# leggedrobotics/wild_visual_navigation

Measured on AMD Instinct MI355X. Metric: frames/sec (448x448 DINO-ViT-S/8 + seg + MLP train-step), higher is better.
Workload: dtype fp16 + e5m2-MX-correction linears (a w = a_h w_h + 2^-12 (a_h8 w_l8 + a_l8 w_h8); ~16 significand bits per product) + f16 attention products (two-plane q in the first six blocks), fp32 accumulate / residual (<= 1e-3 parity mode)

## Files before the change

include/wvn_hip.h:

```cpp
#ifndef WVN_HIP_H
#define WVN_HIP_H
#include <stddef.h>
#ifdef __cplusplus
extern "C" {
#endif

#define WVN_MAX_DEPTH 32
#define WVN_PREC_F32 0
#define WVN_PREC_BF16 1
#define WVN_PREC_X3 2
#define WVN_PREC_FP8 3
#define WVN_PREC_F16 4

#define WVN_PREC_MIX 5

int wvn_version(void);

#define WVN_VIT_MLP_FUSED 1
#define WVN_VIT_QKV_FUSED 2
#define WVN_VIT_FUSE_ANY_SIZE 4
#define WVN_VIT_NO_PROJ_IN_MLP 8
#define WVN_VIT_NO_LN_HANDOVER 16
#define WVN_VIT_NO_A384_X3 32
#define WVN_VIT_X3_NO_A384 64
// ... 302 lines not shown

size_t wvn_rnvp_train_param_count(const wvn_rnvp_desc* d);
size_t wvn_rnvp_train_workspace_bytes(const wvn_rnvp_desc* d, long long R);
size_t wvn_rnvp_train_pack_bytes(const wvn_rnvp_desc* d);
int wvn_rnvp_train_pack(const wvn_rnvp_desc* d, const float* params, const void* packed, void* train_packed, void* stream);
int wvn_rnvp_train_phase_a(const wvn_rnvp_desc* d, const void* packed, const float* x, int ldx, long long R, float* score,
                           double* stats, void* workspace, size_t workspace_bytes, void* stream);
int wvn_rnvp_train_phase_b(const wvn_rnvp_desc* d, const void* packed, const void* train_packed, long long R, const double* stats,
                           float* grads, void* workspace, size_t workspace_bytes, void* stream);
int wvn_rnvp_train_phase_c(const wvn_rnvp_desc* d, float* params, const float* grads, float* adam_m, float* adam_v, int step, float lr,
                           const double* stats, int method, double* conf_state, float* losses, const float* mask,
                           const long long* perm, void* packed, void* train_packed, void* stream);

size_t wvn_segment_predict_workspace_bytes(const wvn_mlp_desc* d, int B, int S);
int wvn_segment_predict(const wvn_mlp_desc* d, const float* params, const float* feat, int ld_row, long long ld_frame,
                        int B, int S, const void* seg, int seg_bytes, int H, int W, float mean, float std, float std_factor,
                        const float* conf_state, float* trav, float* conf, float* loss_reco, void* workspace,
                        size_t workspace_bytes, void* stream);

size_t wvn_wire_bytes(int H, int W, int S, int D);
int wvn_wire_pack(const void* seg, int seg_is_i64, const float* feat, int ldf, void* out, int H, int W, int S, int D, void* stream);
int wvn_wire_unpack(const void* in, long long* seg_i64, int* seg_i32, float* feat, int H, int W, int S, int D, void* stream);

int wvn_debug_gemm_bf16_timed(const void* A, int lda, const void* W, int ldw, const float* bias, void* C, int ldc, int M,
                              int N, int K, int epi, long long* dbg, void* stream);
int wvn_debug_gemm_a384_x3(const void* A, const void* A_lo, int lda, const void* W, const void* W_lo, const float* bias, void* C,
                           void* C_lo, int ldc, int M, int N, int epi, long long* dbg, void* stream);
int wvn_debug_gemm_n384_x3(const void* A, const void* A_lo, int lda, const void* W, const void* W_lo, const float* bias, const float* ls,
                           float* C, int ldc, int M, int K, long long* dbg, void* stream);
int wvn_debug_mlp_x3_frag(const void* xn, const void* xn_lo, const void* W1, const void* W1_lo, const float* b1, void* hid, void* hid_lo,
                          const void* W2p, const float* b2, float* x, int M, int F, long long* dbg1, long long* dbg2, void* stream);
int wvn_debug_gemm_n384_mx(const void* A_h, const void* A_l8, const void* A_h8, const void* Wp, const float* bias, const float* ls, float* C,
                           int ldc, int M, int K, long long* dbg, void* stream);
int wvn_debug_mlp_mx(const float* x, int ldx, const float* ln_stats, const float* ln_g, const float* ln_b, const void* W1p, const float* b1,
                     void* hid_h, void* hid_l8, void* hid_h8, const void* W2p, const float* b2, float* xout, int M, int F, long long* dbg1,
                     long long* dbg2, void* stream);
int wvn_debug_qkv_mx(const float* x, int ldx, const float* ln_stats, const float* ln_g, const float* ln_b, const void* Wp, const float* bias, void* q,
                     void* q_lo, void* k, void* vt, int heads, int npad, int ntok_s, float q_scale, int M, long long* dbg, void* stream);
int wvn_debug_stego_head_fused(const float* x, int ldx, const float* stats, const float* ln_g, const float* ln_b, const void* w_cat, const float* b_cat,
                               void* hid, void* hid_lo, float* code, int ld_code, int frames, int npatch, int ntok_s, void* stream);
int wvn_debug_f16_saturate(const float* in, void* out_f16, int n, void* stream);
int wvn_debug_attention_timing(long long* dbg);
int wvn_debug_attention_variant(int variant);
int wvn_debug_attention_planes(const void* q, const void* q_lo, const void* k, const void* vt, void* out, void* out_lo, int B, int heads,
                               int ntok, int ntok_s, int npad, int out_frag, int qsplit_form, void* stream);
int wvn_debug_n384_pair(int on);
int wvn_debug_kmeans_assign_form(int form);
int wvn_debug_kmeans_linear_rows(int rows);

int wvn_debug_kmeans_screen_stats(unsigned long long* out, int reset);
int wvn_debug_qkv_fused_timing(long long* dbg);
int wvn_debug_mlp_fused_timing(long long* dbg);
int wvn_debug_gemm_n384(const void* A, int lda, const void* W, int ldw, const float* bias, float* C, int ldc, int M, int K,
                        void* stream);


size_t wvn_dense_crf_workspace_bytes(int B, int H, int W, int K);
int wvn_dense_crf(const float* logits1, int K1, long long s1b, long long s1c, long long s1p, const float* logits2, int K2, long long s2b,
                  long long s2c, long long s2p, const unsigned char* image, int B, int H, int W, int iterations, float pos_w, float pos_xy_std,
                  float bi_w, float bi_xy_std, float bi_rgb_std, int* labels, int* nseg_last, float* probs, float* debug, void* workspace,
                  size_t workspace_bytes, void* stream);
int wvn_crf_image(const void* frame, int frame_u8, int B, int src_h, int src_w, const int* rows, const int* cols, int out_h, int out_w,
                  unsigned char* out, void* stream);

size_t wvn_dense_crf_permutohedral_workspace_bytes(int B, int H, int W, int K);
int wvn_dense_crf_permutohedral(const float* logits1, int K1, long long s1b, long long s1c, long long s1p, const float* logits2, int K2,
// ... 14 lines not shown
```

wild_visual_navigation_amd/_lib.py:

```python
import ctypes as C
import os
import threading

import torch

_HERE = os.path.dirname(os.path.abspath(__file__))
LIB_PATH = os.environ.get("WVN_LIB_PATH") or os.path.join(_HERE, "lib", "libwvn_hip.so")
if os.environ.get("WVN_LIB_PATH"):
    import sys as _sys

    print(f"[wild_visual_navigation_amd] WVN_LIB_PATH is set: loading {LIB_PATH} instead of the in-tree build", file=_sys.stderr)

WVN_MAX_DEPTH = 32
PREC_F32, PREC_BF16, PREC_X3, PREC_FP8, PREC_F16, PREC_MIX = 0, 1, 2, 3, 4, 5
VIT_MLP_FUSED = 1
VIT_QKV_FUSED = 2
VIT_FUSE_ANY_SIZE = 4
VIT_NO_PROJ_IN_MLP = 8
VIT_NO_LN_HANDOVER = 16
VIT_NO_A384_X3 = 32
VIT_NO_MX = 1024


def vit_qsplit_blocks(n: int) -> int:
# ... 50 lines not shown


class RnvpDesc(C.Structure):
    _fields_ = [("D", C.c_int), ("h", C.c_int), ("flows", C.c_int)]


MLP_KIND_DOUBLE = 1


_lib = None
_lock = threading.Lock()

_i, _f, _p, _ll, _sz = C.c_int, C.c_float, C.c_void_p, C.c_longlong, C.c_size_t
_SIGNATURES = {
    "wvn_version": ([], _i),
    "wvn_vit_workspace_bytes": ([_p, _i], _sz),
    "wvn_vit_forward": ([_p, _p, _i, _p, _p, _i, _p, _sz, _p], _i),
    "wvn_vit_forward_u8": ([_p, _p, _i, _p, _p, _i, _p, _sz, _p], _i),
    "wvn_vit_forward_frames": ([_p, _p, _i, _i, _i, _p, _p, _i, _p, _p, _i, _p, _sz, _p], _i),
    "wvn_vit_forward_frames_pair": ([_p, _p, _i, _i, _i, _p, _p, _p, _i, _p, _p, _i, _p, _sz, _p], _i),
    "wvn_vit_forward_frames_head": ([_p, _p, _i, _i, _i, _p, _p, _p, _i, _p, _p, _sz, _p], _i),
    "wvn_debug_stego_head_fused": ([_p, _i, _p, _p, _p, _p, _p, _p, _p, _p, _i, _i, _i, _i, _p], _i),
    "wvn_resize_nearest_crop": ([_p, _p, _ll, _i, _i, _p, _p, _i, _i, _i, _p], _i),
    "wvn_prof_enable": ([_i], _i),
    "wvn_prof_collect": ([_p, _p], _i),
    "wvn_gemm_bf16": ([_p, _i, _p, _i, _p, _p, _i, _i, _i, _i, _i, _p], _i),
    "wvn_debug_attention_variant": ([_i], _i),
    "wvn_debug_attention_planes": ([_p, _p, _p, _p, _p, _p, _i, _i, _i, _i, _i, _i, _i, _p], _i),
    "wvn_debug_kmeans_assign_form": ([_i], _i),
    "wvn_debug_kmeans_screen_stats": ([_p, _i], _i),
    "wvn_debug_mlp_x3_frag": ([_p, _p, _p, _p, _p, _p, _p, _p, _p, _p, _i, _i, _p, _p, _p], _i),
    "wvn_debug_gemm_n384_x3": ([_p, _p, _i, _p, _p, _p, _p, _p, _i, _i, _i, _p, _p], _i),
    "wvn_debug_gemm_n384_mx": ([_p, _p, _p, _p, _p, _p, _p, _i, _i, _i, _p, _p], _i),
    "wvn_debug_mlp_mx": ([_p, _i, _p, _p, _p, _p, _p, _p, _p, _p, _p, _p, _p, _i, _i, _p, _p, _p], _i),
    "wvn_debug_qkv_mx": ([_p, _i, _p, _p, _p, _p, _p, _p, _p, _p, _p, _i, _i, _i, _f, _i, _p, _p], _i),
    "wvn_debug_gemm_a384_x3": ([_p, _p, _i, _p, _p, _p, _p, _p, _i, _i, _i, _i, _p, _p], _i),
    "wvn_stream_create_cu_mask": ([_p, _p, _i], _i),
    "wvn_stream_destroy": ([_p], _i),
    "wvn_debug_qkv_fused_timing": ([_p], _i),
    "wvn_debug_mlp_fused_timing": ([_p], _i),
    "wvn_qkv_fused": ([_p, _i, _p, _p, _f, _p, _p, _p, _p, _p, _i, _i, _i, _f, _i, _p], _i),
    "wvn_proj_mlp_fused": ([_p, _i, _p, _p, _p, _p, _p, _f, _p, _p, _p, _p, _p, _p, _i, _i, _i, _p], _i),
    "wvn_mlp_fused": ([_p, _i, _p, _p, _f, _p, _p, _p, _p, _p, _p, _i, _i, _i, _p], _i),
    "wvn_gemm_f16": ([_p, _i, _p, _i, _p, _p, _i, _i, _i, _i, _i, _p], _i),
    "wvn_qkv_fused_f16": ([_p, _i, _p, _p, _f, _p, _p, _p, _p, _p, _i, _i, _i, _f, _i, _p], _i),
    "wvn_proj_mlp_resident": ([_p, _i, _p, _p, _p, _p, _f, _p, _p, _p, _p, _p, _i, _i, _i, _p, _p, _f, _p, _p], _i),
    "wvn_proj_mlp_resident_f16": ([_p, _i, _p, _p, _p, _p, _f, _p, _p, _p, _p, _p, _i, _i, _i, _p, _p, _f, _p, _p], _i),
    "wvn_qkv_prenorm": ([_p, _p, _p, _p, _p, _p, _i, _i, _i, _f, _i, _p], _i),
    "wvn_qkv_prenorm_f16": ([_p, _p, _p, _p, _p, _p, _i, _i, _i, _f, _i, _p], _i),
    "wvn_proj_mlp_fused_f16": ([_p, _i, _p, _p, _p, _p, _p, _f, _p, _p, _p, _p, _p, _p, _i, _i, _i, _p], _i),
    "wvn_mlp_fused_f16": ([_p, _i, _p, _p, _f, _p, _p, _p, _p, _p, _p, _i, _i, _i, _p], _i),
    "wvn_attention_f16": ([_p, _p, _p, _p, _i, _i, _i, _i, _f, _p], _i),
    "wvn_gemm_x3": ([_p, _p, _i, _p, _p, _i, _p, _p, _p, _i, _i, _i, _i, _i, _p], _i),
    "wvn_quantize_rows_fp8": ([_p, _i, _i, _p, _i, _p, _i, _i, _p], _i),
    "wvn_layernorm_fp8": ([_p, _p, _p, _p, _i, _p, _i, _i, _f, _p], _i),
    "wvn_gemm_fp8": ([_p, _i, _p, _i, _p, _p, _p, _p, _i, _i, _i, _i, _i, _p], _i),
    "wvn_gemm_a768_fp8": ([_p, _i, _p, _p, _p, _p, _p, _p, _i, _i, _i, _i, _p, _p, _p, _i, _i, _i, _f, _p], _i),
    "wvn_gemm_fp8_mx": ([_p, _i, _p, _p, _i, _p, _p, _p, _p, _i, _i, _i, _i, _i, _p], _i),
    "wvn_split_planes": ([_p, _i, _p, _p, _i, _i, _i, _p], _i),
    "wvn_attention_x3": ([_p, _p, _p, _p, _p, _p, _p, _p, _i, _i, _i, _i, _f, _p], _i),
    "wvn_gemm_f32": ([_p, _i, _i, _p, _i, _i, _p, _p, _i, _i, _i, _i, _i, _p, _i, _p], _i),
    "wvn_layernorm": ([_p, _p, _p, _p, _i, _i, _i, _f, _p], _i),
    "wvn_attention_bf16": ([_p, _p, _p, _p, _i, _i, _i, _i, _f, _p], _i),
    "wvn_attention_f32": ([_p, _p, _p, _p, _i, _i, _i, _i, _f, _p], _i),
    "wvn_patchify": ([_p, _p, _i, _i, _i, _i, _p], _i),
    "wvn_patchify_u8": ([_p, _p, _i, _i, _i, _p], _i),
# ... 127 lines not shown
```

wild_visual_navigation_amd/csrc/api.hip:

```cpp
#include <math.h>
#include <string.h>

#include "../../include/wvn_hip.h"

#include "common.h"
#include "wvn_internal.h"

#define RET_IF(x)            \
  do {                       \
    int rc__ = (x);          \
    if (rc__ != WVN_OK) return rc__; \
  } while (0)

extern "C" {

int wvn_version(void) { return 101; }

size_t wvn_vit_workspace_bytes(const wvn_vit_model* m, int batch) {
  if (!m || batch <= 0) return 0;
  return wvn_vit_workspace_bytes_impl(m, batch);
}

int wvn_vit_forward(const wvn_vit_model* m, const float* img, int batch, float* tokens_f32, void* tokens_lowp,
                    int ld_lowp, void* workspace, size_t workspace_bytes, void* stream) {
// ... 190 lines not shown
int wvn_debug_qkv_fused_timing(long long* dbg) { g_qkv_fused_dbg = dbg; return WVN_OK; }
int wvn_stream_create_cu_mask(void** stream, const unsigned int* mask, int words) {
  if (!stream || !mask || words <= 0) return WVN_ERR_ARG;
  hipStream_t st = nullptr;
  const hipError_t e = hipExtStreamCreateWithCUMask(&st, (uint32_t)words, mask);
  if (e != hipSuccess) return (int)e;
  *stream = (void*)st;
  return WVN_OK;
}
int wvn_stream_destroy(void* stream) {
  if (!stream) return WVN_ERR_ARG;
  const hipError_t e = hipStreamDestroy((hipStream_t)stream);
  return e == hipSuccess ? WVN_OK : (int)e;
}

int wvn_debug_gemm_a384_x3(const void* A, const void* A_lo, int lda, const void* W, const void* W_lo, const float* bias, void* C,
                           void* C_lo, int ldc, int M, int N, int epi, long long* dbg, void* stream) {
  if (epi != EPI_GELU_BF16 && epi != EPI_RESID_F32) return WVN_ERR_ARG;
  return wvn_gemm_a384_x3_launch(wvn_desc_a384(A, A_lo, lda, W, W_lo, bias, C, C_lo, ldc, M, N, dbg), epi, (hipStream_t)stream);
}
int wvn_debug_gemm_n384_x3(const void* A, const void* A_lo, int lda, const void* W, const void* W_lo, const float* bias, const float* ls,
                           float* C, int ldc, int M, int K, long long* dbg, void* stream) {
  return wvn_gemm_n384_x3_launch(wvn_desc_n384(A, A_lo, lda, W, W_lo, bias, ls, C, ldc, M, K, nullptr, dbg), EPI_RESID_F32, (hipStream_t)stream);
}
int wvn_debug_mlp_x3_frag(const void* xn, const void* xn_lo, const void* W1, const void* W1_lo, const float* b1, void* hid, void* hid_lo,
                          const void* W2p, const float* b2, float* x, int M, int F, long long* dbg1, long long* dbg2, void* stream) {
  RET_IF(wvn_gemm_a384_x3_launch(wvn_desc_a384(xn, xn_lo, 384, W1, W1_lo, b1, hid, hid_lo, F, M, F, dbg1), EPI_GELU_FRAG, (hipStream_t)stream));
  return wvn_gemm_n384_x3_frag_launch(wvn_desc_n384(hid, hid_lo, F, W2p, nullptr, b2, nullptr, x, 384, M, F, nullptr, dbg2), EPI_RESID_F32, (hipStream_t)stream);
}
int wvn_debug_gemm_n384_mx(const void* A_h, const void* A_l8, const void* A_h8, const void* Wp, const float* bias, const float* ls, float* C,
                           int ldc, int M, int K, long long* dbg, void* stream) {
  return wvn_gemm_n384_mx_launch(wvn_desc_n384(A_h, A_l8, K, Wp, nullptr, bias, ls, C, ldc, M, K, nullptr, dbg, A_h8), EPI_RESID_F32, (hipStream_t)stream);
}
int wvn_debug_mlp_mx(const float* x, int ldx, const float* ln_stats, const float* ln_g, const float* ln_b, const void* W1p, const float* b1,
                     void* hid_h, void* hid_l8, void* hid_h8, const void* W2p, const float* b2, float* xout, int M, int F, long long* dbg1,
                     long long* dbg2, void* stream) {
  GemmBf16Params p1 = wvn_desc_a384(nullptr, nullptr, 0, W1p, nullptr, b1, hid_h, hid_l8, F, M, F, dbg1, hid_h8);
  wvn_desc_ln_on_load(p1, x, ldx, ln_stats, ln_g, ln_b);
  RET_IF(wvn_gemm_a384_mx_launch(p1, EPI_GELU_FRAG, (hipStream_t)stream));
  if (!W2p) return WVN_OK;
  return wvn_gemm_n384_mx_launch(wvn_desc_n384(hid_h, hid_l8, F, W2p, nullptr, b2, nullptr, xout, 384, M, F, nullptr, dbg2, hid_h8), EPI_RESID_F32, (hipStream_t)stream);
}
int wvn_debug_qkv_mx(const float* x, int ldx, const float* ln_stats, const float* ln_g, const float* ln_b, const void* Wp, const float* bias, void* q,
                     void* q_lo, void* k, void* vt, int heads, int npad, int ntok_s, float q_scale, int M, long long* dbg, void* stream) {
  GemmBf16Params p = wvn_desc_a384(nullptr, nullptr, 0, Wp, nullptr, bias, nullptr, nullptr, 0, M, 3 * heads * 64, dbg);
  wvn_desc_ln_on_load(p, x, ldx, ln_stats, ln_g, ln_b);
  wvn_desc_qkv_epilogue(p, q, k, vt, heads, npad, 0, ntok_s, q_scale, 1, q_lo);
  return wvn_gemm_a384_mx_launch(p, EPI_QKV, (hipStream_t)stream);
}
int wvn_debug_n384_pair(int on) {
  if (on >= 32) { wvn_gemm_a384_mx_set_form(on - 32); return WVN_OK; }
  wvn_gemm_n384_x3_set_pair(on);
  return WVN_OK;
}
int wvn_debug_kmeans_screen_stats(unsigned long long* out, int reset) { return out ? wvn_kmeans_pixels_screen_stats(out, reset) : WVN_ERR_ARG; }
int wvn_debug_kmeans_assign_form(int form) { wvn_kmeans_pixels_set_assign_form(form); return WVN_OK; }
int wvn_debug_attention_variant(int v) { wvn_attention_bf16_set_variant(v); wvn_attention_bf16_set_variant_f16(v); return WVN_OK; }
int wvn_debug_attention_planes(const void* q, const void* q_lo, const void* k, const void* vt, void* out, void* out_lo, int B, int heads, int ntok,
                               int ntok_s, int npad, int out_frag, int qsplit_form, void* stream) {
  if (!q || !k || !vt || !out || B < 1 || heads < 1 || ntok < 1 || ntok_s < ntok || ntok_s > npad) return WVN_ERR_ARG;
  if (qsplit_form < 0 || qsplit_form > 2 || (qsplit_form == 0) != (q_lo == nullptr)) return WVN_ERR_ARG;
  if (out_frag < 0 || out_frag > 2 || (out_frag != 0 && (!out_lo || heads != 6))) return WVN_ERR_ARG;
  return wvn_attention_bf16_launch_f16((const bf16_t*)q, (const bf16_t*)k, (const bf16_t*)vt, (bf16_t*)out, B, heads, ntok, ntok_s, npad, 0.f,
                                       (hipStream_t)stream, (bf16_t*)out_lo, (const bf16_t*)q_lo, out_frag, qsplit_form);
}

int wvn_debug_gemm_bf16_timed(const void* A, int lda, const void* W, int ldw, const float* bias, void* C, int ldc, int M,
                              int N, int K, int epi, long long* dbg, void* stream) {
  if (epi < 0 || epi > EPI_ACCUM_F32 || !C) return WVN_ERR_ARG;
  GemmBf16Params p{};
  p.A = (const bf16_t*)A; p.lda = lda; p.W = (const bf16_t*)W; p.ldw = ldw; p.bias = bias; p.C = C; p.ldc = ldc;
  p.M = M; p.N = N; p.K = K; p.dbg = dbg;
  return wvn_gemm_bf16_launch(p, epi, (hipStream_t)stream);
}

int wvn_debug_gemm_n384(const void* A, int lda, const void* W, int ldw, const float* bias, float* C, int ldc, int M, int K,
                        void* stream) {
  GemmBf16Params p{};
  p.A = (const bf16_t*)A; p.lda = lda; p.W = (const bf16_t*)W; p.ldw = ldw; p.bias = bias; p.C = C; p.ldc = ldc;
  p.M = M; p.N = 384; p.K = K;
  return wvn_gemm_n384_launch(p, EPI_RESID_F32, (hipStream_t)stream, nullptr, 1);
}

// ... 583 lines not shown
```

wild_visual_navigation_amd/csrc/gemm_n384_x3.hip:

```cpp
#include <type_traits>

#include "common.h"
#include "wvn_internal.h"

namespace {

constexpr int NN = 384;
constexpr int NTILE = NN / 32;
constexpr int BKS = 16;
constexpr int BM = 128;
constexpr int NS = 4;
constexpr int W_PLANE = NN * BKS * 2;
constexpr int A_PLANE = BM * BKS * 2;
constexpr int A_OFF = 2 * W_PLANE;
constexpr int STAGE_BYTES = 2 * W_PLANE + 2 * A_PLANE;
constexpr int RING_BYTES = NS * STAGE_BYTES;
constexpr int STG_PITCH = 132;
constexpr int STG_BYTES = 32 * STG_PITCH * 4;
constexpr int BIAS_OFF = RING_BYTES;
constexpr int LS_OFF = BIAS_OFF + NN * 4;
constexpr int LDS_BYTES = LS_OFF + NN * 4;
constexpr int WP = 6, AP = 2;

struct N384X3Params {
// ... 529 lines not shown
            __builtin_amdgcn_sched_group_barrier(0x008, 1, 0);
            __builtin_amdgcn_sched_group_barrier(0x100, 1, 0);
            __builtin_amdgcn_sched_group_barrier(0x010, 1, 0);
            __builtin_amdgcn_sched_group_barrier(0x002, 2, 0);
          }
          __builtin_amdgcn_sched_barrier(0);
        }
        if (i + PD < nk) load_a(i + PD, jj);
        __builtin_amdgcn_sched_barrier(0);
        if constexpr (TIMING) { t_wait += c1 - c0; t_steps += (long long)__builtin_amdgcn_s_memtime() - c1; }
      }
    }
    long long e0 = 0;
    if constexpr (TIMING) e0 = (long long)__builtin_amdgcn_s_memtime();
    asm volatile("s_waitcnt vmcnt(0)" ::: "memory");
    n384_pair_epilogue(acc, smem, wave, lane, rg, ch, m0w, rs_c, p.ldc, bias_l, ls_l, p.stats, p.eps, p.M);
    if constexpr (TIMING) t_epi += (long long)__builtin_amdgcn_s_memtime() - e0;
  }
  if constexpr (TIMING) {
    if (lane == 0 && p.dbg && ch == 0) {
      long long* d = p.dbg + ((size_t)blockIdx.x * 4 + rg) * 4;
      d[0] = t_wait; d[1] = t_steps; d[2] = t_epi; d[3] = (long long)__builtin_amdgcn_s_memtime() - t_start;
    }
  }
}

typedef __attribute__((ext_vector_type(8))) int i32x8_t;
typedef __attribute__((ext_vector_type(8))) _Float16 f16x8_t;
constexpr int MXD = 2;
constexpr int MX_SC_ONE = 0x7f7f7f7f, MX_SC_RES = 0x73737373;

struct N384MXExtra { unsigned a_l8_off; };

template <bool TIMING, int VAR = 0>
__global__ __launch_bounds__(512, 1) void gemm_n384_mx_pair_kernel(N384X3Params p, N384MXExtra ex) {
  wvn_fp16_saturate();
  extern __shared__ __attribute__((aligned(16))) unsigned char smem[];
  const int tid = threadIdx.x, lane = tid & 63;
  const int wave = __builtin_amdgcn_readfirstlane(tid >> 6);
  const int rg = wave & 3, ch = wave >> 2;
  const int l31 = lane & 31, hi = lane >> 5;
  const int nk = p.K / BKS;
  const int nmac = p.K / 64;
  const float* bias_l = (const float*)(smem + PBIAS_OFF);
  const float* ls_l = (const float*)(smem + PLS_OFF);
  for (int i = tid; i < NN; i += 512) {
    ((float*)(smem + PBIAS_OFF))[i] = p.bias ? p.bias[i] : 0.f;
    ((float*)(smem + PLS_OFF))[i] = p.ls ? p.ls[i] : 1.f;
  }
  const __amdgpu_buffer_rsrc_t rs_w = __builtin_amdgcn_make_buffer_rsrc((void*)p.W, 0, (unsigned)((size_t)4 * NN * p.K), 0x00020000);
  const size_t mpad = (size_t)(p.M + 31) / 32 * 32;
  const __amdgpu_buffer_rsrc_t rs_a = __builtin_amdgcn_make_buffer_rsrc((void*)p.A, 0, (unsigned)(ex.a_l8_off + mpad * p.K), 0x00020000);
  const __amdgpu_buffer_rsrc_t rs_c = __builtin_amdgcn_make_buffer_rsrc((void*)p.C, 0, (unsigned)((size_t)p.M * p.ldc * 4), 0x00020000);
  const unsigned wv0 = (unsigned)(wave * PFW * 1024 + lane * 16);
  const unsigned rdw = l31 * 32 + ((hi ^ ((l31 >> 3) & 1)) << 4) + ch * 6 * 1024;

  long long t_wait = 0, t_steps = 0, t_epi = 0;
  const long long t_start = TIMING ? (long long)__builtin_amdgcn_s_memtime() : 0;
  const int nrb = (p.M + BM - 1) / BM;
  for (int rb = blockIdx.x; rb < nrb; rb += gridDim.x) {
    const int m0w = rb * BM + rg * 32;
    const unsigned a_base = __builtin_amdgcn_readfirstlane((unsigned)((size_t)(m0w >> 5) * p.K * 64));
    const unsigned a8_base = __builtin_amdgcn_readfirstlane((unsigned)((size_t)(m0w >> 5) * p.K * 32));
    auto piece_w = [&](int i, int u) {
      unsigned char* st = smem + (i % PNS) * FSTAGE;
      __builtin_amdgcn_raw_ptr_buffer_load_lds(rs_w, (__attribute__((address_space(3))) void*)(st + (wave * PFW + u) * 1024), 16, wv0 + u * 1024,
                                               __builtin_amdgcn_readfirstlane((unsigned)i * FSTAGE), 0, 0);
    };
    u32x4_t ah[MXD][4], a8[MXD][2][2];
    auto load_ah = [&](int c, int slot) {
#pragma unroll
      for (int s = 0; s < 4; ++s)
        ah[slot][s] = __builtin_amdgcn_raw_buffer_load_b128(rs_a, lane * 16, __builtin_amdgcn_readfirstlane(a_base + (unsigned)(c * 4 + s) * 1024), 0);
    };
    auto load_a8 = [&](int c, int slot) {
#pragma unroll
      for (int x = 0; x < 2; ++x)
        a8[slot][1][x] = __builtin_amdgcn_raw_buffer_load_b128(rs_a, lane * 16, __builtin_amdgcn_readfirstlane(a8_base + ex.a_l8_off + (unsigned)(c * 2 + x) * 1024), 0);
    };
    auto derive_h8 = [&](int slot) {
      typedef __attribute__((ext_vector_type(2))) short s16x2_t;
      typedef __attribute__((ext_vector_type(2))) _Float16 h2_t;
#pragma unroll
      for (int sfr = 0; sfr < 4; ++sfr) {
        uint32_t d[2] = {0, 0};
#pragma unroll
        for (int e = 0; e < 4; ++e) {
          const uint32_t pr = ah[slot][sfr][e];
          const s16x2_t o = __builtin_bit_cast(s16x2_t, d[e >> 1]);
          d[e >> 1] = __builtin_bit_cast(uint32_t, (e & 1) ? __builtin_amdgcn_cvt_scalef32_pk_bf8_f16(o, __builtin_bit_cast(h2_t, pr), 1.0f, true)
                                                           : __builtin_amdgcn_cvt_scalef32_pk_bf8_f16(o, __builtin_bit_cast(h2_t, pr), 1.0f, false));
        }
        a8[slot][0][sfr >> 1][2 * (sfr & 1)] = d[0];
        a8[slot][0][sfr >> 1][2 * (sfr & 1) + 1] = d[1];
      }
    };
    __syncthreads();
#pragma unroll
    for (int c = 0; c < MXD; ++c) {
      load_ah(c, c);
      __builtin_amdgcn_sched_barrier(0);
      load_a8(c, c);
      __builtin_amdgcn_sched_barrier(0);
    }
#pragma unroll
    for (int i0 = 0; i0 < PNS - 1; ++i0)
      if (i0 < nk) {
#pragma unroll
        for (int u = 0; u < PFW; ++u) piece_w(i0, u);
      }

    f32x16_t acc[NTILE / 2];
#pragma unroll
    for (int t = 0; t < NTILE / 2; ++t)
#pragma unroll
      for (int r = 0; r < 16; ++r) acc[t][r] = 0.f;

    u32x4_t wq[2][2][2];
    asm volatile("s_waitcnt vmcnt(%0)" ::"n"((PNS - 2) * PFW) : "memory");
    __builtin_amdgcn_s_barrier();
#pragma unroll
    for (int x = 0; x < 2; ++x)
#pragma unroll
      for (int t = 0; t < 2; ++t) wq[0][x][t] = *(const u32x4_t*)(smem + rdw + x * W_PLANE + t * 1024);
    for (int ib = 0; ib < nk; ib += 4 * MXD) {
#pragma unroll
      for (int jj = 0; jj < 4 * MXD; ++jj) {
        const int i = ib + jj;
        const int kind = jj & 3, slot = jj >> 2;
        long long c0 = 0, c1 = 0;
        if constexpr (TIMING) c0 = (long long)__builtin_amdgcn_s_memtime();
        if constexpr (VAR != 4) {
          constexpr int W3 = (PNS - 3) * PFW;
          if (jj == 0) { if (i == 0) asm volatile("s_waitcnt vmcnt(%0)" ::"n"(W3) : "memory"); else asm volatile("s_waitcnt vmcnt(%0)" ::"n"(W3 + 6) : "memory"); }
          else if (jj == 1) { if (i == 1) asm volatile("s_waitcnt vmcnt(%0)" ::"n"(W3) : "memory"); else asm volatile("s_waitcnt vmcnt(%0)" ::"n"(W3 + 2) : "memory"); }
          else if (jj == 2) { if (i == 2) asm volatile("s_waitcnt vmcnt(%0)" ::"n"(W3 + 4) : "memory"); else asm volatile("s_waitcnt vmcnt(%0)" ::"n"(W3 + 6) : "memory"); }
          else if ((jj & 3) == 0) asm volatile("s_waitcnt vmcnt(%0)" ::"n"(W3 + 6) : "memory");
          else if ((jj & 3) == 1) asm volatile("s_waitcnt vmcnt(%0)" ::"n"(W3 + 2) : "memory");
          else if ((jj & 3) == 2) asm volatile("s_waitcnt vmcnt(%0)" ::"n"(W3 + 6) : "memory");
          else asm volatile("s_waitcnt vmcnt(%0)" ::"n"(W3 + 4) : "memory");
          __builtin_amdgcn_s_barrier();
        }
        if constexpr (TIMING) c1 = (long long)__builtin_amdgcn_s_memtime();
        __builtin_amdgcn_sched_barrier(0);
        const unsigned char* st = smem + (i % PNS) * FSTAGE;
        const unsigned char* st1 = smem + ((i + 1) % PNS) * FSTAGE;
        const int s0 = jj & 1;
#pragma unroll
        for (int pr = 0; pr < NTILE / 4; ++pr) {
          const int cur = (s0 + pr) & 1, nx = cur ^ 1;
          if constexpr (!(VAR & 1) || VAR == 4) piece_w(i + PNS - 1, pr);
          const unsigned char* src = pr + 1 < NTILE / 4 ? st + (2 * pr + 2) * 1024 : st1;
#pragma unroll
          for (int x = 0; x < 2; ++x)
#pragma unroll
            for (int t = 0; t < 2; ++t) wq[nx][x][t] = *(const u32x4_t*)(src + rdw + x * W_PLANE + t * 1024);
          if (kind == 1 && pr == 0) derive_h8(slot);
          if (kind < 2) {
// ... 1 lines not shown
            for (int x = 0; x < 2; ++x)
#pragma unroll
              for (int t = 0; t < 2; ++t)
                acc[2 * pr + t] = __builtin_amdgcn_mfma_f32_32x32x16_f16(__builtin_bit_cast(f16x8_t, wq[cur][x][t]), __builtin_bit_cast(f16x8_t, ah[slot][2 * kind + x]),
                                                                         acc[2 * pr + t], 0, 0, 0);
#pragma unroll
            for (int n = 0; n < 4; ++n) {
              __builtin_amdgcn_sched_group_barrier(0x008, 1, 0);
              __builtin_amdgcn_sched_group_barrier(0x100, 1, 0);
              __builtin_amdgcn_sched_group_barrier(0x010, 1, 0);
              __builtin_amdgcn_sched_group_barrier(0x002, 2, 0);
            }
          } else {
            const u32x4_t a0 = a8[slot][kind - 2][0], a1 = a8[slot][kind - 2][1];
            const i32x8_t av = {(int)a0[0], (int)a0[1], (int)a0[2], (int)a0[3], (int)a1[0], (int)a1[1], (int)a1[2], (int)a1[3]};
#pragma unroll
            for (int t = 0; t < 2; ++t) {
              const u32x4_t w0 = wq[cur][0][t], w1 = wq[cur][1][t];
              const i32x8_t wv = {(int)w0[0], (int)w0[1], (int)w0[2], (int)w0[3], (int)w1[0], (int)w1[1], (int)w1[2], (int)w1[3]};
              acc[2 * pr + t] = __builtin_amdgcn_mfma_scale_f32_32x32x64_f8f6f4(wv, av, acc[2 * pr + t], 1, 1, 0, kind == 2 ? MX_SC_RES : MX_SC_ONE, 0,
                                                                                kind == 2 ? MX_SC_ONE : MX_SC_RES);
            }
#pragma unroll
            for (int n = 0; n < 2; ++n) {
              __builtin_amdgcn_sched_group_barrier(0x008, 1, 0);
              __builtin_amdgcn_sched_group_barrier(0x100, 2, 0);
              __builtin_amdgcn_sched_group_barrier(0x010, 1, 0);
              __builtin_amdgcn_sched_group_barrier(0x002, 4, 0);
            }
          }
          __builtin_amdgcn_sched_barrier(0);
        }
        const int c2 = (i >> 2) + MXD;
        if constexpr (!(VAR & 2) || VAR == 4) {
          if (kind == 1) load_ah(c2, slot);
          if (kind == 3) load_a8(c2, slot);
        }
        __builtin_amdgcn_sched_barrier(0);
        if constexpr (TIMING) { t_wait += c1 - c0; t_steps += (long long)__builtin_amdgcn_s_memtime() - c1; }
      }
    }
    long long e0 = 0;
    if constexpr (TIMING) e0 = (long long)__builtin_amdgcn_s_memtime();
    asm volatile("s_waitcnt vmcnt(0)" ::: "memory");
    n384_pair_epilogue(acc, smem, wave, lane, rg, ch, m0w, rs_c, p.ldc, bias_l, ls_l, p.stats, p.eps, p.M);
    if constexpr (TIMING) t_epi += (long long)__builtin_amdgcn_s_memtime() - e0;
  }
  if constexpr (TIMING) {
    if (lane == 0 && p.dbg && ch == 0) {
      long long* d = p.dbg + ((size_t)blockIdx.x * 4 + rg) * 4;
      d[0] = t_wait; d[1] = t_steps; d[2] = t_epi; d[3] = (long long)__builtin_amdgcn_s_memtime() - t_start;
    }
  }
}

int g_n384_mx_var = 0;
int g_n384_pair = 1;

int n384x3_num_cus() {
  static int n = 0;
  if (n == 0) {
    int dev = 0;
    hipDeviceProp_t prop;
    if (hipGetDevice(&dev) == hipSuccess && hipGetDeviceProperties(&prop, dev) == hipSuccess) n = prop.multiProcessorCount;
    if (n <= 0) n = 256;
  }
  return n;
}

}

int wvn_gemm_n384_x3_launch(const GemmBf16Params& g, int epi, hipStream_t st) {
  const bool patch = epi == EPI_PATCH;
  if (epi != EPI_RESID_F32 && epi != EPI_ACCUM_F32 && !patch) return WVN_ERR_ARG;
  if (patch && (!g.pos || g.npatch <= 0 || (g.npatch & 1) || g.ntok_s < g.npatch + 1 || g.ldc != NN || g.ls || (g.M % g.npatch) != 0)) return WVN_ERR_ARG;
  if (g.N != NN || g.K <= 0 || (g.K % BKS) != 0 || g.M <= 0 || !g.A || !g.A_lo || !g.W || !g.W_lo || !g.C) return WVN_ERR_ARG;
  if ((g.lda % 8) || (g.ldw % 8) || (g.ldc % 4) || g.ldw != g.K) return WVN_ERR_ARG;
  if (((uintptr_t)g.A | (uintptr_t)g.A_lo | (uintptr_t)g.W | (uintptr_t)g.W_lo | (uintptr_t)g.C) & 15) return WVN_ERR_ARG;
  if (g.A_lo <= g.A || g.W_lo <= g.W) return WVN_ERR_ARG;
  const size_t a_plane = (size_t)(g.A_lo - g.A), w_plane = (size_t)(g.W_lo - g.W);
  const size_t c_rows = patch ? (size_t)(g.M / g.npatch) * g.ntok_s : (size_t)g.M;
  if ((a_plane + (size_t)g.M * g.lda) * 2 >= (1ull << 32) || c_rows * g.ldc * 4 >= (1ull << 32) || (w_plane + (size_t)NN * g.ldw) * 2 >= (1ull << 32))
    return WVN_ERR_ARG;
  N384X3Params p{};
  p.A = g.A; p.a_plane = a_plane; p.lda = g.lda; p.W = g.W; p.w_plane = w_plane; p.ldw = g.ldw; p.bias = g.bias; p.ls = g.ls;
  p.C = (float*)g.C; p.ldc = g.ldc; p.M = g.M; p.K = g.K; p.dbg = g.dbg; p.stats = g.ln_stats_out; p.eps = g.ln_eps;
  if (patch) { p.pos = g.pos; p.npatch = g.npatch; p.ntok_s = g.ntok_s; p.c_rows = (int)c_rows; p.stats = nullptr; }
  static LdsOptIn lds_opt_in;
// ... 15 lines not shown
  if ((a_plane + mpad * g.K) * 2 >= (1ull << 32) || (size_t)g.M * g.ldc * 4 >= (1ull << 32) || (size_t)2 * NN * g.K * 2 >= (1ull << 31)) return WVN_ERR_ARG;
  N384X3Params p{};
  p.A = g.A; p.a_plane = a_plane; p.lda = g.K; p.W = g.W; p.w_plane = 0; p.ldw = g.K; p.bias = g.bias; p.ls = g.ls;
  p.C = (float*)g.C; p.ldc = g.ldc; p.M = g.M; p.K = g.K; p.dbg = g.dbg; p.stats = g.ln_stats_out; p.eps = g.ln_eps;
  static LdsOptIn lds_opt_in;
  if (const int rc = lds_opt_in(PAIR_LDS_BYTES, (const void*)gemm_n384_x3_frag_kernel<false>, (const void*)gemm_n384_x3_frag_kernel<true>,
                                (const void*)gemm_n384_x3_frag_pair_kernel<false>, (const void*)gemm_n384_x3_frag_pair_kernel<true>)) return rc;
  const int ncu = n384x3_num_cus(), nrb = ceil_div(g.M, BM);
  const int grid = nrb < ncu ? nrb : ncu;
  if (g_n384_pair) {
    if (p.dbg) hipLaunchKernelGGL(gemm_n384_x3_frag_pair_kernel<true>, dim3(grid), dim3(512), PAIR_LDS_BYTES, st, p);
    else hipLaunchKernelGGL(gemm_n384_x3_frag_pair_kernel<false>, dim3(grid), dim3(512), PAIR_LDS_BYTES, st, p);
  } else if (p.dbg) hipLaunchKernelGGL(gemm_n384_x3_frag_kernel<true>, dim3(grid), dim3(256), LDS_BYTES, st, p);
  else hipLaunchKernelGGL(gemm_n384_x3_frag_kernel<false>, dim3(grid), dim3(256), LDS_BYTES, st, p);
  WVN_LAUNCH_CHECK();
  return WVN_OK;
}
int wvn_gemm_n384_mx_launch(const GemmBf16Params& g, int epi, hipStream_t st) {
  if (epi != EPI_RESID_F32 && epi != EPI_ACCUM_F32) return WVN_ERR_ARG;
  if (g.N != NN || g.K <= 0 || (g.K % 128) != 0 || g.M <= 0 || !g.A || !g.A_lo || !g.W || !g.C || (g.ldc % 4)) return WVN_ERR_ARG;
  if (((uintptr_t)g.A | (uintptr_t)g.A_lo | (uintptr_t)g.W | (uintptr_t)g.C) & 15) return WVN_ERR_ARG;
  const size_t mpad = (size_t)(g.M + 31) / 32 * 32;
  const uintptr_t a0 = (uintptr_t)g.A, al = (uintptr_t)g.A_lo;
  if (al < a0 + mpad * g.K * 2) return WVN_ERR_ARG;
  const uintptr_t top = al + mpad * g.K;
  if (top - a0 >= (1ull << 32) || (size_t)g.M * g.ldc * 4 >= (1ull << 32) || (size_t)4 * NN * g.K >= (1ull << 31)) return WVN_ERR_ARG;
  N384X3Params p{};
  p.A = g.A; p.a_plane = 0; p.lda = g.K; p.W = g.W; p.w_plane = 0; p.ldw = g.K; p.bias = g.bias; p.ls = g.ls;
  p.C = (float*)g.C; p.ldc = g.ldc; p.M = g.M; p.K = g.K; p.dbg = g.dbg; p.stats = g.ln_stats_out; p.eps = g.ln_eps;
  N384MXExtra ex{(unsigned)(al - a0)};
  static LdsOptIn lds_opt_in;
  if (const int rc = lds_opt_in(PAIR_LDS_BYTES, (const void*)gemm_n384_mx_pair_kernel<false>, (const void*)gemm_n384_mx_pair_kernel<true>,
                                (const void*)gemm_n384_mx_pair_kernel<true, 1>, (const void*)gemm_n384_mx_pair_kernel<true, 2>,
                                (const void*)gemm_n384_mx_pair_kernel<true, 3>, (const void*)gemm_n384_mx_pair_kernel<true, 4>)) return rc;
  const int ncu = n384x3_num_cus(), nrb = ceil_div(g.M, BM);
  const int grid = nrb < ncu ? nrb : ncu;
  if (p.dbg && g_n384_mx_var == 1) hipLaunchKernelGGL((gemm_n384_mx_pair_kernel<true, 1>), dim3(grid), dim3(512), PAIR_LDS_BYTES, st, p, ex);
  else if (p.dbg && g_n384_mx_var == 2) hipLaunchKernelGGL((gemm_n384_mx_pair_kernel<true, 2>), dim3(grid), dim3(512), PAIR_LDS_BYTES, st, p, ex);
  else if (p.dbg && g_n384_mx_var == 3) hipLaunchKernelGGL((gemm_n384_mx_pair_kernel<true, 3>), dim3(grid), dim3(512), PAIR_LDS_BYTES, st, p, ex);
  else if (p.dbg && g_n384_mx_var == 4) hipLaunchKernelGGL((gemm_n384_mx_pair_kernel<true, 4>), dim3(grid), dim3(512), PAIR_LDS_BYTES, st, p, ex);
  else if (p.dbg) hipLaunchKernelGGL(gemm_n384_mx_pair_kernel<true>, dim3(grid), dim3(512), PAIR_LDS_BYTES, st, p, ex);
  else hipLaunchKernelGGL(gemm_n384_mx_pair_kernel<false>, dim3(grid), dim3(512), PAIR_LDS_BYTES, st, p, ex);
  WVN_LAUNCH_CHECK();
  return WVN_OK;
}
void wvn_gemm_n384_x3_set_pair(int on) {
  if (on >= 16) { g_n384_mx_var = on - 16; return; }
  g_n384_pair = on ? 1 : 0;
}
```

Before: 884.2.

## Prefetch residual rows into A-operand registers during last K trip of n384 MX GEMM

Adds a BND variant of the n384 MX pair GEMM, enabled by default. It peels the final K trip and, in place of the now-unneeded A-operand prefetches, issues loads of the fp32 residual tile into the freed register slots. The remaining residual rows are loaded before a partial vmcnt wait, and a new epilogue adds bias, layer scale and residual from registers, then computes the LN statistics. The goal is to hide residual read latency behind the last MFMA steps, at the cost of more register pressure and extra code complexity.

```diff
diff --git a/include/wvn_hip.h b/include/wvn_hip.h
--- a/include/wvn_hip.h
+++ b/include/wvn_hip.h
@@ -358,6 +358,8 @@
                           const void* W2p, const float* b2, float* x, int M, int F, long long* dbg1, long long* dbg2, void* stream);
 int wvn_debug_gemm_n384_mx(const void* A_h, const void* A_l8, const void* A_h8, const void* Wp, const float* bias, const float* ls, float* C,
                            int ldc, int M, int K, long long* dbg, void* stream);
+int wvn_debug_gemm_n384_mx_stats(const void* A_h, const void* A_l8, const void* Wp, const float* bias, const float* ls, float* C, int ldc, int M,
+                                 int K, float* ln_stats_out, long long* dbg, void* stream);
 int wvn_debug_mlp_mx(const float* x, int ldx, const float* ln_stats, const float* ln_g, const float* ln_b, const void* W1p, const float* b1,
                      void* hid_h, void* hid_l8, void* hid_h8, const void* W2p, const float* b2, float* xout, int M, int F, long long* dbg1,
                      long long* dbg2, void* stream);
diff --git a/wild_visual_navigation_amd/_lib.py b/wild_visual_navigation_amd/_lib.py
--- a/wild_visual_navigation_amd/_lib.py
+++ b/wild_visual_navigation_amd/_lib.py
@@ -106,6 +106,7 @@
     "wvn_debug_mlp_x3_frag": ([_p, _p, _p, _p, _p, _p, _p, _p, _p, _p, _i, _i, _p, _p, _p], _i),
     "wvn_debug_gemm_n384_x3": ([_p, _p, _i, _p, _p, _p, _p, _p, _i, _i, _i, _p, _p], _i),
     "wvn_debug_gemm_n384_mx": ([_p, _p, _p, _p, _p, _p, _p, _i, _i, _i, _p, _p], _i),
+    "wvn_debug_gemm_n384_mx_stats": ([_p, _p, _p, _p, _p, _p, _i, _i, _i, _p, _p, _p], _i),
     "wvn_debug_mlp_mx": ([_p, _i, _p, _p, _p, _p, _p, _p, _p, _p, _p, _p, _p, _i, _i, _p, _p, _p], _i),
     "wvn_debug_qkv_mx": ([_p, _i, _p, _p, _p, _p, _p, _p, _p, _p, _p, _i, _i, _i, _f, _i, _p, _p], _i),
     "wvn_debug_gemm_a384_x3": ([_p, _p, _i, _p, _p, _p, _p, _p, _i, _i, _i, _i, _p, _p], _i),
diff --git a/wild_visual_navigation_amd/csrc/api.hip b/wild_visual_navigation_amd/csrc/api.hip
--- a/wild_visual_navigation_amd/csrc/api.hip
+++ b/wild_visual_navigation_amd/csrc/api.hip
@@ -246,6 +246,10 @@
                            int ldc, int M, int K, long long* dbg, void* stream) {
   return wvn_gemm_n384_mx_launch(wvn_desc_n384(A_h, A_l8, K, Wp, nullptr, bias, ls, C, ldc, M, K, nullptr, dbg, A_h8), EPI_RESID_F32, (hipStream_t)stream);
 }
+int wvn_debug_gemm_n384_mx_stats(const void* A_h, const void* A_l8, const void* Wp, const float* bias, const float* ls, float* C, int ldc, int M, int K,
+                                 float* ln_stats_out, long long* dbg, void* stream) {
+  return wvn_gemm_n384_mx_launch(wvn_desc_n384(A_h, A_l8, K, Wp, nullptr, bias, ls, C, ldc, M, K, ln_stats_out, dbg), EPI_RESID_F32, (hipStream_t)stream);
+}
 int wvn_debug_mlp_mx(const float* x, int ldx, const float* ln_stats, const float* ln_g, const float* ln_b, const void* W1p, const float* b1,
                      void* hid_h, void* hid_l8, void* hid_h8, const void* W2p, const float* b2, float* xout, int M, int F, long long* dbg1,
                      long long* dbg2, void* stream) {
@@ -263,6 +267,7 @@
   return wvn_gemm_a384_mx_launch(p, EPI_QKV, (hipStream_t)stream);
 }
 int wvn_debug_n384_pair(int on) {
+  if (on >= 48) { wvn_gemm_n384_x3_set_pair(on); return WVN_OK; }
   if (on >= 32) { wvn_gemm_a384_mx_set_form(on - 32); return WVN_OK; }
   wvn_gemm_n384_x3_set_pair(on);
   return WVN_OK;
diff --git a/wild_visual_navigation_amd/csrc/gemm_n384_x3.hip b/wild_visual_navigation_amd/csrc/gemm_n384_x3.hip
--- a/wild_visual_navigation_amd/csrc/gemm_n384_x3.hip
+++ b/wild_visual_navigation_amd/csrc/gemm_n384_x3.hip
@@ -585,7 +585,78 @@
 
 struct N384MXExtra { unsigned a_l8_off; };
 
-template <bool TIMING, int VAR = 0>
+__device__ __forceinline__ void n384_mx_pair_epilogue(const f32x16_t (&acc)[NTILE / 2], const u32x4_t (&r)[24], unsigned res_base, unsigned ldc16, unsigned char* smem,
+                                                      int wave, int lane, int rg, int ch, int m0w, __amdgpu_buffer_rsrc_t rs_c, unsigned cvoff,
+                                                      const float* bias_l, const float* ls_l, float* stats, float eps, int M) {
+  const int l31 = lane & 31, hi = lane >> 5, l15 = lane & 15, rq = lane >> 4;
+  asm volatile("s_waitcnt lgkmcnt(0)" ::: "memory");
+  __builtin_amdgcn_s_barrier();
+  asm volatile("" ::: "memory");
+  __builtin_amdgcn_sched_barrier(0);
+  float* stg = (float*)(smem + wave * PSTG_BYTES);
+  const int col0 = 192 * ch;
+  float s1[8], s2[8];
+#pragma unroll
+  for (int it = 0; it < 8; ++it) { s1[it] = 0.f; s2[it] = 0.f; }
+#pragma unroll
+  for (int c = 0; c < 3; ++c) {
+#pragma unroll
+    for (int tt = 0; tt < 2; ++tt)
+#pragma unroll
+      for (int g = 0; g < 4; ++g) {
+        const f32x16_t& a = acc[2 * c + tt];
+        const f32x4_t o = {a[4 * g], a[4 * g + 1], a[4 * g + 2], a[4 * g + 3]};
+        *(f32x4_t*)(stg + l31 * PSTG_PITCH + 32 * tt + 8 * g + 4 * hi) = o;
+      }
+    const f32x4_t b4 = *(const f32x4_t*)(bias_l + col0 + 64 * c + l15 * 4);
+    const f32x4_t l4 = *(const f32x4_t*)(ls_l + col0 + 64 * c + l15 * 4);
+#pragma unroll
+    for (int it = 0; it < 8; ++it) {
+      const f32x4_t v = *(const f32x4_t*)(stg + (4 * it + rq) * PSTG_PITCH + l15 * 4);
+      u32x4_t o;
+#pragma unroll
+      for (int e = 0; e < 4; ++e) {
+        const float y = (v[e] + b4[e]) * l4[e] + __uint_as_float(r[8 * c + it][e]);
+        o[e] = __float_as_uint(y);
+        s1[it] += y;
+        s2[it] = fmaf(y, y, s2[it]);
+      }
+      wvn_store_b128_guarded(o, rs_c, cvoff, __builtin_amdgcn_readfirstlane(res_base + (unsigned)it * ldc16 + (unsigned)c * 256u));
+    }
+  }
+  if (stats) {
+    float* sx = (float*)(smem + PSTAT_OFF);
+    auto dpp_add = [](float v, auto ctrl) {
+      constexpr int C = decltype(ctrl)::value;
+      return v + __builtin_bit_cast(float, __builtin_amdgcn_update_dpp(0, __builtin_bit_cast(int, v), C, 0xf, 0xf, false));
+    };
+#pragma unroll
+    for (int it = 0; it < 8; ++it) {
+      float a = s1[it], b = s2[it];
+      a = dpp_add(a, std::integral_constant<int, 0xB1>{}); b = dpp_add(b, std::integral_constant<int, 0xB1>{});
+      a = dpp_add(a, std::integral_constant<int, 0x4E>{}); b = dpp_add(b, std::integral_constant<int, 0x4E>{});
+      a = dpp_add(a, std::integral_constant<int, 0x141>{}); b = dpp_add(b, std::integral_constant<int, 0x141>{});
+      a = dpp_add(a, std::integral_constant<int, 0x140>{}); b = dpp_add(b, std::integral_constant<int, 0x140>{});
+      if (l15 == 0) *(wvn_f32x2_t*)(sx + ((size_t)ch * BM + rg * 32 + 4 * it + rq) * 2) = wvn_f32x2_t{a, b};
+    }
+    asm volatile("s_waitcnt lgkmcnt(0)" ::: "memory");
+    __builtin_amdgcn_s_barrier();
+    asm volatile("" ::: "memory");
+    __builtin_amdgcn_sched_barrier(0);
+    if (ch == 0 && lane < 32) {
+      const int m = m0w + lane;
+      if (m < M) {
+        const wvn_f32x2_t p0 = *(const wvn_f32x2_t*)(sx + ((size_t)rg * 32 + lane) * 2), p1 = *(const wvn_f32x2_t*)(sx + ((size_t)BM + rg * 32 + lane) * 2);
+        const float a = p0[0] + p1[0], b = p0[1] + p1[1];
+        const float mean = a * (1.0f / NN);
+        const float var = fmaxf(b * (1.0f / NN) - mean * mean, 0.f);
+        *(wvn_f32x2_t*)(stats + 2 * (size_t)m) = wvn_f32x2_t{mean, 1.0f / sqrtf(var + eps)};
+      }
+    }
+  }
+}
+
+template <bool TIMING, int VAR = 0, int BND = 0>
 __global__ __launch_bounds__(512, 1) void gemm_n384_mx_pair_kernel(N384X3Params p, N384MXExtra ex) {
   wvn_fp16_saturate();
   extern __shared__ __attribute__((aligned(16))) unsigned char smem[];
@@ -611,10 +682,14 @@
   long long t_wait = 0, t_steps = 0, t_epi = 0;
   const long long t_start = TIMING ? (long long)__builtin_amdgcn_s_memtime() : 0;
   const int nrb = (p.M + BM - 1) / BM;
+  const unsigned cvoff = (unsigned)((((lane >> 4) * p.ldc + (lane & 15) * 4) * 4));
+  const unsigned ldc16 = (unsigned)(p.ldc * 16);
   for (int rb = blockIdx.x; rb < nrb; rb += gridDim.x) {
     const int m0w = rb * BM + rg * 32;
     const unsigned a_base = __builtin_amdgcn_readfirstlane((unsigned)((size_t)(m0w >> 5) * p.K * 64));
     const unsigned a8_base = __builtin_amdgcn_readfirstlane((unsigned)((size_t)(m0w >> 5) * p.K * 32));
+    const unsigned res_base = __builtin_amdgcn_readfirstlane((unsigned)((m0w * p.ldc + 192 * ch) * 4));
+    auto res_so = [&](int idx) { return __builtin_amdgcn_readfirstlane(res_base + (unsigned)(idx & 7) * ldc16 + (unsigned)(idx >> 3) * 256u); };
     auto piece_w = [&](int i, int u) {
       unsigned char* st = smem + (i % PNS) * FSTAGE;
       __builtin_amdgcn_raw_ptr_buffer_load_lds(rs_w, (__attribute__((address_space(3))) void*)(st + (wave * PFW + u) * 1024), 16, wv0 + u * 1024,
@@ -676,7 +751,8 @@
     for (int x = 0; x < 2; ++x)
 #pragma unroll
       for (int t = 0; t < 2; ++t) wq[0][x][t] = *(const u32x4_t*)(smem + rdw + x * W_PLANE + t * 1024);
-    for (int ib = 0; ib < nk; ib += 4 * MXD) {
+    auto trip = [&](const int ib, auto last_c) {
+      constexpr bool last = decltype(last_c)::value;
 #pragma unroll
       for (int jj = 0; jj < 4 * MXD; ++jj) {
         const int i = ib + jj;
@@ -744,18 +820,49 @@
           __builtin_amdgcn_sched_barrier(0);
         }
         const int c2 = (i >> 2) + MXD;
-        if constexpr (!(VAR & 2) || VAR == 4) {
+        if constexpr (last) {
+          if (kind == 1) {
+#pragma unroll
+            for (int s = 0; s < 4; ++s) ah[slot][s] = __builtin_amdgcn_raw_buffer_load_b128(rs_c, cvoff, res_so(6 * slot + s), 0);
+          }
+          if (kind == 3) {
+#pragma unroll
+            for (int x = 0; x < 2; ++x) a8[slot][1][x] = __builtin_amdgcn_raw_buffer_load_b128(rs_c, cvoff, res_so(6 * slot + 4 + x), 0);
+          }
+        } else if constexpr (!(VAR & 2) || VAR == 4) {
           if (kind == 1) load_ah(c2, slot);
           if (kind == 3) load_a8(c2, slot);
         }
         __builtin_amdgcn_sched_barrier(0);
         if constexpr (TIMING) { t_wait += c1 - c0; t_steps += (long long)__builtin_amdgcn_s_memtime() - c1; }
       }
+    };
+    if constexpr (BND >= 1) {
+      for (int ib = 0; ib < nk - 4 * MXD; ib += 4 * MXD) trip(ib, std::false_type{});
+      trip(nk - 4 * MXD, std::true_type{});
+    } else {
+      for (int ib = 0; ib < nk; ib += 4 * MXD) trip(ib, std::false_type{});
     }
     long long e0 = 0;
     if constexpr (TIMING) e0 = (long long)__builtin_amdgcn_s_memtime();
-    asm volatile("s_waitcnt vmcnt(0)" ::: "memory");
-    n384_pair_epilogue(acc, smem, wave, lane, rg, ch, m0w, rs_c, p.ldc, bias_l, ls_l, p.stats, p.eps, p.M);
+    if constexpr (BND >= 1) {
+      u32x4_t r[24];
+#pragma unroll
+      for (int slot = 0; slot < MXD; ++slot) {
+#pragma unroll
+        for (int s = 0; s < 4; ++s) r[6 * slot + s] = ah[slot][s];
+#pragma unroll
+        for (int x = 0; x < 2; ++x) r[6 * slot + 4 + x] = a8[slot][1][x];
+      }
+#pragma unroll
+      for (int idx = 6 * MXD; idx < 24; ++idx) r[idx] = __builtin_amdgcn_raw_buffer_load_b128(rs_c, cvoff, res_so(idx), 0);
+      __builtin_amdgcn_sched_barrier(0);
+      asm volatile("s_waitcnt vmcnt(%0)" ::"n"(24 - 6 * MXD) : "memory");
+      n384_mx_pair_epilogue(acc, r, res_base, ldc16, smem, wave, lane, rg, ch, m0w, rs_c, cvoff, bias_l, ls_l, p.stats, p.eps, p.M);
+    } else {
+      asm volatile("s_waitcnt vmcnt(0)" ::: "memory");
+      n384_pair_epilogue(acc, smem, wave, lane, rg, ch, m0w, rs_c, p.ldc, bias_l, ls_l, p.stats, p.eps, p.M);
+    }
     if constexpr (TIMING) t_epi += (long long)__builtin_amdgcn_s_memtime() - e0;
   }
   if constexpr (TIMING) {
@@ -766,6 +873,7 @@
   }
 }
 
+int g_n384_mx_bnd = 1;
 int g_n384_mx_var = 0;
 int g_n384_pair = 1;
 
@@ -847,19 +955,23 @@
   static LdsOptIn lds_opt_in;
   if (const int rc = lds_opt_in(PAIR_LDS_BYTES, (const void*)gemm_n384_mx_pair_kernel<false>, (const void*)gemm_n384_mx_pair_kernel<true>,
                                 (const void*)gemm_n384_mx_pair_kernel<true, 1>, (const void*)gemm_n384_mx_pair_kernel<true, 2>,
-                                (const void*)gemm_n384_mx_pair_kernel<true, 3>, (const void*)gemm_n384_mx_pair_kernel<true, 4>)) return rc;
+                                (const void*)gemm_n384_mx_pair_kernel<true, 3>, (const void*)gemm_n384_mx_pair_kernel<true, 4>,
+                                (const void*)gemm_n384_mx_pair_kernel<false, 0, 1>, (const void*)gemm_n384_mx_pair_kernel<true, 0, 1>)) return rc;
   const int ncu = n384x3_num_cus(), nrb = ceil_div(g.M, BM);
   const int grid = nrb < ncu ? nrb : ncu;
   if (p.dbg && g_n384_mx_var == 1) hipLaunchKernelGGL((gemm_n384_mx_pair_kernel<true, 1>), dim3(grid), dim3(512), PAIR_LDS_BYTES, st, p, ex);
   else if (p.dbg && g_n384_mx_var == 2) hipLaunchKernelGGL((gemm_n384_mx_pair_kernel<true, 2>), dim3(grid), dim3(512), PAIR_LDS_BYTES, st, p, ex);
   else if (p.dbg && g_n384_mx_var == 3) hipLaunchKernelGGL((gemm_n384_mx_pair_kernel<true, 3>), dim3(grid), dim3(512), PAIR_LDS_BYTES, st, p, ex);
   else if (p.dbg && g_n384_mx_var == 4) hipLaunchKernelGGL((gemm_n384_mx_pair_kernel<true, 4>), dim3(grid), dim3(512), PAIR_LDS_BYTES, st, p, ex);
+  else if (p.dbg && g_n384_mx_bnd == 1) hipLaunchKernelGGL((gemm_n384_mx_pair_kernel<true, 0, 1>), dim3(grid), dim3(512), PAIR_LDS_BYTES, st, p, ex);
   else if (p.dbg) hipLaunchKernelGGL(gemm_n384_mx_pair_kernel<true>, dim3(grid), dim3(512), PAIR_LDS_BYTES, st, p, ex);
+  else if (g_n384_mx_bnd == 1) hipLaunchKernelGGL((gemm_n384_mx_pair_kernel<false, 0, 1>), dim3(grid), dim3(512), PAIR_LDS_BYTES, st, p, ex);
   else hipLaunchKernelGGL(gemm_n384_mx_pair_kernel<false>, dim3(grid), dim3(512), PAIR_LDS_BYTES, st, p, ex);
   WVN_LAUNCH_CHECK();
   return WVN_OK;
 }
 void wvn_gemm_n384_x3_set_pair(int on) {
+  if (on >= 48) { g_n384_mx_bnd = on == 48 ? 0 : 1; return; }
   if (on >= 16) { g_n384_mx_var = on - 16; return; }
   g_n384_pair = on ? 1 : 0;
 }
```

Result: no change. 889.9, median of 6 (+0.6%).
